# Cathoven-AI/Montreal-Forced-Aligner

Measured on AMD Instinct MI355X. Metric: aligned utterances/sec (whole node), 10 s utts, 5k-state triphone, higher is better.
Workload: dtype f32 scores from 2-way f16-split products (3*2^-22 per term worst case), f64 path costs

## Files before the change

montreal_forced_aligner_amd/csrc/feats.hip:

```cpp
#include <algorithm>
#include <cstdlib>

#include "ctx.hpp"

namespace {

constexpr int kTile = 64;
constexpr int kMaxDim = 16;
constexpr int kMaxOut = 64;
constexpr size_t kMaxLdsBytes = 64 << 10;

__global__ __launch_bounds__(256) void cmvn_utt_kernel(const float *__restrict__ feats, const int64_t *__restrict__ frame_off,
                                                       int dim, double *__restrict__ partial) {
  __shared__ double sx[16][kMaxDim], sxx[16][kMaxDim];
  const int utt = blockIdx.x, d = threadIdx.x & 15, s = threadIdx.x >> 4;
  const int64_t f0 = frame_off[utt];
  const int T = (int)(frame_off[utt + 1] - f0);
  double a = 0.0, b = 0.0;
  if (d < dim)
    for (int t = s; t < T; t += 16) {
      float x = feats[(f0 + t) * dim + d];
      a += (double)x;
      b += (double)(x * x);
    }
// ... 73 lines not shown
      int level = c / p.dim, d = c % p.dim;
      float acc = 0.0f;
      const float *xc = x + (r + halo) * p.dim + d;
      if (level == 0) acc = fmaf(1.0f, xc[0], acc);
      else if (level == 1) {
#pragma unroll
        for (int j = -2; j <= 2; j++) {
          int tf = t + j; tf = tf < 0 ? 0 : (tf >= T ? T - 1 : tf);
          float s = kDelta1[j + 2];
          if (s != 0.0f) acc = fmaf(s, xc[(tf - t) * p.dim], acc);
        }
      } else {
#pragma unroll
        for (int j = -4; j <= 4; j++) {
          int tf = t + j; tf = tf < 0 ? 0 : (tf >= T ? T - 1 : tf);
          float s = kDelta2[j + 4];
          if (s != 0.0f) acc = fmaf(s, xc[(tf - t) * p.dim], acc);
        }
      }
      p.out[(f0 + t) * od + c] = acc;
    }
    return;
  }
  const int nsp = 2 * p.ctx + 1, sdim = nsp * p.dim;
  const bool lda_offset = (p.lda_cols == sdim + 1);
  for (int i = threadIdx.x; i < kTile * p.lda_rows; i += blockDim.x) {
    int r = i / p.lda_rows, o = i % p.lda_rows, t = t0 + r;
    if (t >= T) continue;
    const float *m = mat + o * p.lda_cols;
    float acc = 0.0f;
    for (int j = 0; j < nsp; j++) {
      int tf = t + j - p.ctx; tf = tf < 0 ? 0 : (tf >= T ? T - 1 : tf);
      const float *xr = x + (tf - t0 + halo) * p.dim;
      for (int d = 0; d < p.dim; d++) acc = fmaf(m[j * p.dim + d], xr[d], acc);
    }
    if (lda_offset) acc += m[sdim];
    if (p.fmllr) y[r * p.lda_rows + o] = acc;
    else p.out[(f0 + t) * p.lda_rows + o] = acc;
  }
  if (!p.fmllr) return;
  __syncthreads();
  const float *fm = mat + p.lda_rows * p.lda_cols;
  for (int i = threadIdx.x; i < kTile * p.lda_rows; i += blockDim.x) {
    int r = i / p.lda_rows, o = i % p.lda_rows, t = t0 + r;
    if (t >= T) continue;
    const float *m = fm + o * (p.lda_rows + 1);
    float acc = 0.0f;
    for (int d = 0; d < p.lda_rows; d++) acc = fmaf(m[d], y[r * p.lda_rows + d], acc);
    acc += m[p.lda_rows];
    p.out[(f0 + t) * p.lda_rows + o] = acc;
  }
}

constexpr int kTileLda = 128;
template <int kDim, int kCtx, int kR>
__global__ __launch_bounds__(256) void feats_lda_kernel(FeatParams p) {
  extern __shared__ __attribute__((aligned(16))) float smem[];
  constexpr int kSdim = (2 * kCtx + 1) * kDim;
  constexpr int kXS = (kDim + 3) & ~3;
  static_assert(kR % 4 == 0, "LDA output rows are read 16 bytes at a time");
  const int utt = blockIdx.y;
  const int64_t f0 = p.frame_off[utt];
  const int T = (int)(p.frame_off[utt + 1] - f0);
  const int t0 = blockIdx.x * kTileLda;
  if (t0 >= T) return;
  constexpr int halo = kCtx, rows = kTileLda + 2 * halo;
  constexpr int R = kR;
  float *X = smem;
  constexpr int x_floats = rows * kXS > R * (R + 1) ? rows * kXS : R * (R + 1);
  float *Y = X + x_floats;
  const int spk = p.utt2spk ? p.utt2spk[utt] : 0;
  for (int i = threadIdx.x; i < rows * kDim; i += blockDim.x) {
    int r = i / kDim, d = i % kDim;
    int t = t0 - halo + r;
    t = t < 0 ? 0 : (t >= T ? T - 1 : t);
    float v = p.mfcc[(f0 + t) * kDim + d];
    if (p.cmvn) {
      const double *st = p.cmvn + (size_t)spk * 2 * (kDim + 1);
      v += (float)(-(st[d] / st[kDim]));
    }
    X[r * kXS + d] = v;
  }
  for (int i = threadIdx.x; i < R * p.lda_cols; i += blockDim.x) Y[i] = p.lda[i];
  __syncthreads();
  constexpr int G = 256 / R;
  const int o = threadIdx.x % R, g = threadIdx.x / R;
  const bool active = g < G;
  const bool lda_offset = (p.lda_cols == kSdim + 1);
  float m[kSdim];
#pragma unroll
  for (int k = 0; k < kSdim; k++) m[k] = Y[o * p.lda_cols + k];
  const float m_off = lda_offset ? Y[o * p.lda_cols + kSdim] : 0.0f;
  __syncthreads();
  if (active) {
    for (int r = g; r < kTileLda; r += 2 * G) {
      const int t = t0 + r;
      if (t >= T) break;
      const int r2 = r + G;
      const bool two = r2 < kTileLda && t0 + r2 < T;
      const float *xa = X + r * kXS;
      const float *xb = X + (two ? r2 : r) * kXS;
      float acc = 0.0f, acc2 = 0.0f;
#pragma unroll
      for (int j = 0; j < 2 * kCtx + 1; j++) {
        const float *xr = xa + j * kXS, *xr2 = xb + j * kXS;
#pragma unroll
        for (int d4 = 0; d4 + 4 <= kDim; d4 += 4) {
          const float4 x4 = *reinterpret_cast<const float4 *>(xr + d4);
          const float4 y4 = *reinterpret_cast<const float4 *>(xr2 + d4);
          acc = fmaf(m[j * kDim + d4], x4.x, acc);      acc2 = fmaf(m[j * kDim + d4], y4.x, acc2);
          acc = fmaf(m[j * kDim + d4 + 1], x4.y, acc);  acc2 = fmaf(m[j * kDim + d4 + 1], y4.y, acc2);
          acc = fmaf(m[j * kDim + d4 + 2], x4.z, acc);  acc2 = fmaf(m[j * kDim + d4 + 2], y4.z, acc2);
          acc = fmaf(m[j * kDim + d4 + 3], x4.w, acc);  acc2 = fmaf(m[j * kDim + d4 + 3], y4.w, acc2);
        }
#pragma unroll
        for (int d = kDim & ~3; d < kDim; d++) { acc = fmaf(m[j * kDim + d], xr[d], acc); acc2 = fmaf(m[j * kDim + d], xr2[d], acc2); }
      }
      if (lda_offset) { acc += m_off; acc2 += m_off; }
      if (p.fmllr) { Y[r * R + o] = acc; if (two) Y[r2 * R + o] = acc2; }
      else { p.out[(f0 + t) * R + o] = acc; if (two) p.out[(f0 + t0 + r2) * R + o] = acc2; }
    }
  }
  if (!p.fmllr) return;
  __syncthreads();
  const float *fm = p.fmllr + (size_t)spk * R * (R + 1);
  for (int i = threadIdx.x; i < R * (R + 1); i += blockDim.x) X[i] = fm[i];
  __syncthreads();
  if (!active) return;
  float f[kR];
#pragma unroll
  for (int k = 0; k < kR; k++) f[k] = X[o * (R + 1) + k];
  const float f_off = X[o * (R + 1) + R];
  for (int r = g; r < kTileLda; r += 2 * G) {
    const int t = t0 + r;
    if (t >= T) break;
    const int r2 = r + G;
    const bool two = r2 < kTileLda && t0 + r2 < T;
    const float *ys = Y + r * R, *ys2 = Y + (two ? r2 : r) * R;
    float acc = 0.0f, acc2 = 0.0f;
#pragma unroll
    for (int k = 0; k < kR; k += 4) {
      const float4 y4 = *reinterpret_cast<const float4 *>(ys + k);
      const float4 z4 = *reinterpret_cast<const float4 *>(ys2 + k);
      acc = fmaf(f[k], y4.x, acc);          acc2 = fmaf(f[k], z4.x, acc2);
      acc = fmaf(f[k + 1], y4.y, acc);      acc2 = fmaf(f[k + 1], z4.y, acc2);
      acc = fmaf(f[k + 2], y4.z, acc);      acc2 = fmaf(f[k + 2], z4.z, acc2);
      acc = fmaf(f[k + 3], y4.w, acc);      acc2 = fmaf(f[k + 3], z4.w, acc2);
    }
    acc += f_off; acc2 += f_off;
    p.out[(f0 + t) * R + o] = acc;
    if (two) p.out[(f0 + t0 + r2) * R + o] = acc2;
  }
}

int upload_delta_scales(mfa_ctx *c) {
  MFA_HIP_CHECK(c, hipSetDevice(c->device));
  float s0[1] = {1.0f}, s1[5] = {0}, s2[9] = {0};
  {
    float normalizer = 0.0f;
    for (int j = -2; j <= 2; j++) { normalizer += j * j; s1[j + 2] += (float)j * s0[0]; }
    float sc = (float)(1.0 / normalizer);
    for (float &v : s1) v *= sc;
  }
  {
    float normalizer = 0.0f;
    for (int j = -2; j <= 2; j++) {
      normalizer += j * j;
      for (int k = -2; k <= 2; k++) s2[j + k + 4] += (float)j * s1[k + 2];
    }
    float sc = (float)(1.0 / normalizer);
    for (float &v : s2) v *= sc;
  }
  MFA_HIP_CHECK(c, hipMemcpyToSymbol(HIP_SYMBOL(kDelta1), s1, sizeof(s1)));
  MFA_HIP_CHECK(c, hipMemcpyToSymbol(HIP_SYMBOL(kDelta2), s2, sizeof(s2)));
  return 0;
}

}

extern "C" {

MFA_API int mfa_cmvn_stats(mfa_ctx *c, const float *d_feats, const int64_t *d_frame_off, int32_t n_utt, int32_t dim,
                           const int32_t *d_spk_utt_off, const int32_t *d_spk_utt, int32_t n_spk, double *d_stats) {
  if (dim > kMaxDim) return c->fail("CMVN: feature dim %d > %d", dim, kMaxDim);
  if (n_utt <= 0 || n_spk <= 0) return 0;
  size_t need = (size_t)n_utt * 2 * (dim + 1) * sizeof(double);
  if (c->ws_bytes < need) {
    if (c->d_ws) { MFA_HIP_CHECK(c, hipStreamSynchronize(c->stream)); (void)hipFree(c->d_ws); c->d_ws = nullptr; c->ws_bytes = 0; }
    MFA_HIP_CHECK(c, hipMalloc(&c->d_ws, need));
    c->ws_bytes = need;
  }
  KernelTimer kt(c, MFA_K_CMVN);
  hipLaunchKernelGGL(cmvn_utt_kernel, dim3(n_utt), dim3(256), 0, c->stream, d_feats, d_frame_off, dim, (double *)c->d_ws);
  int total = n_spk * 2 * (dim + 1);
  hipLaunchKernelGGL(cmvn_spk_kernel, dim3((total + 255) / 256), dim3(256), 0, c->stream, (const double *)c->d_ws,
                     d_spk_utt_off, d_spk_utt, n_spk, dim, d_stats);
  MFA_HIP_CHECK(c, hipGetLastError());
  return 0;
}

MFA_API int mfa_feats_batch(mfa_ctx *c, const float *d_mfcc, const int64_t *d_frame_off, int32_t n_utt, int32_t max_frames,
                            int32_t dim, const int32_t *d_utt2spk, const double *d_cmvn, int32_t mode, int32_t splice_ctx,
                            const float *d_lda, int32_t lda_rows, int32_t lda_cols, const float *d_fmllr, float *d_out) {
  if (dim > kMaxDim) return c->fail("feats: base dim %d > %d", dim, kMaxDim);
  if (n_utt <= 0 || max_frames <= 0) return 0;
  if (n_utt > 65535) return c->fail("at most 65535 utterances per feature launch (got %d)", n_utt);
  if (mode != 0 && mode != 1) return c->fail("feats: bad mode %d", mode);
  if (d_cmvn && !d_utt2spk) return c->fail("feats: CMVN given without utt2spk");
  if (!c->delta_uploaded) { if (upload_delta_scales(c)) return -1; c->delta_uploaded = true; }
  FeatParams p;
  p.dim = dim; p.mode = mode; p.ctx = splice_ctx; p.lda_rows = lda_rows; p.lda_cols = lda_cols;
  p.mfcc = d_mfcc; p.frame_off = d_frame_off; p.utt2spk = d_utt2spk; p.cmvn = d_cmvn; p.lda = d_lda; p.fmllr = d_fmllr;
  p.out = d_out;
  constexpr int kDim = 13, kCtx = 3, kR = 40;
  const char *generic = getenv("MFA_FEATS_GENERIC");
  const bool register_rows = mode == 1 && dim == kDim && splice_ctx == kCtx && lda_rows == kR && !(generic && generic[0] == '1');
  size_t lds = 0;
  if (mode == 0) {
    lds = (size_t)(kTile + 8) * dim * 4;
  } else {
    int sdim = (2 * splice_ctx + 1) * dim;
    if (!d_lda || lda_rows <= 0 || lda_rows > kMaxOut || (lda_cols != sdim && lda_cols != sdim + 1))
      return c->fail("feats: LDA %dx%d does not match spliced dim %d", lda_rows, lda_cols, sdim);
    lds = ((size_t)(kTile + 2 * splice_ctx) * dim + (size_t)lda_rows * lda_cols + (size_t)lda_rows * (lda_rows + 1) +
           (size_t)kTile * lda_rows) * 4;
    if (lds > kMaxLdsBytes && !register_rows)
      return c->fail("feats: base dim %d, splice ±%d, LDA %dx%d needs %zu bytes of LDS (a launch may ask for %zu)", dim,
                     splice_ctx, lda_rows, lda_cols, lds, kMaxLdsBytes);
  }
  dim3 grid((max_frames + kTile - 1) / kTile, n_utt);
  KernelTimer kt(c, MFA_K_FEATS);
  if (register_rows) {
    const int rows = kTileLda + 2 * splice_ctx;
    size_t x_floats = std::max((size_t)rows * ((kDim + 3) & ~3), (size_t)lda_rows * (lda_rows + 1));
    size_t y_floats = std::max((size_t)kTileLda * lda_rows, (size_t)lda_rows * lda_cols);
    dim3 grid2((max_frames + kTileLda - 1) / kTileLda, n_utt);
    hipLaunchKernelGGL((feats_lda_kernel<kDim, kCtx, kR>), grid2, dim3(256), (x_floats + y_floats) * 4, c->stream, p);
  } else {
    hipLaunchKernelGGL(feats_kernel, grid, dim3(256), lds, c->stream, p);
  }
  MFA_HIP_CHECK(c, hipGetLastError());
  return 0;
}

}
```

montreal_forced_aligner_amd/csrc/viterbi.hip:

```cpp
#include <cmath>
#include <cstdint>
#include <cstdlib>
#include <cstring>

#include <algorithm>
#include <vector>

#include "ctx.hpp"

namespace {

typedef unsigned long long u64;
typedef unsigned int u32;

constexpr u32 kEmpty = 0xFFFFFFFFu;
constexpr u32 kClaim = 0xFFFFFFFEu;
constexpr u32 kOver = 0xFFFFFFFDu;
constexpr u64 kKeyInf = 0xFFFFFFFFFFFFFFFFull;
constexpr int kMinActive = 20;
constexpr float kBeamDelta = 0.5f;
constexpr float kHashRatio = 2.0f;
constexpr int kArcBits = 6;
constexpr int kMaxArcsPerState = 1 << kArcBits;

// ... 240 lines not shown
    }
  } else {
  {
    u32 pos = bpos;
    for (int c0 = T - 1; c0 >= 0; c0 -= 64) {
      const int tl = c0 - lane;
      const u32 tokv = tl >= 0 ? tokoff[tl] : 0u;
      const int cnt = min(64, c0 + 1);
      for (int k = 0; k < cnt; k++) {
        const u32 to = (u32)__builtin_amdgcn_readlane((int)tokv, k);
        const u64 rec = bp[(u64)to + pos];
        if (lane == 0) ali[c0 - k] = (int32_t)(rec >> 32);
        pos = (u32)(rec & 0xFFFFFFFFu);
      }
    }
  }
  __threadfence_block();
  WSYNC();
  for (int c0 = 0; c0 < T; c0 += 64) {
    const int tt = c0 + lane;
    int arc = tt < T ? ali[tt] : 0;
    int il = 0, ol = 0; float w = 0.0f, ac = 0.0f;
    if (tt < T) {
      il = a_il[arc]; ol = a_ol[arc]; w = a_w[arc];
      ac = -(p.scale * ll[(size_t)tt * P + a_col[arc]]);
    }
    const u64 mask = __ballot(ol != 0);
    if (ol != 0) words[nw_out + __popcll(mask & ((1ull << lane) - 1ull))] = ol;
    nw_out += (u32)__popcll(mask);
    float my_fl = 0.0f;
    const int lim = min(64, T - c0);
    for (int j = 0; j < lim; j++) {
      float wj = __shfl(w, j), acj = __shfl(ac, j);
      double nc = ((double)wj + cost) + (double)acj;
      float tot = (float)(nc - cost);
      float acost = tot - wj;
      w1 += wj; w2 += acost;
      cost = nc;
      if (lane == j) my_fl = acost * inv_scale;
    }
    if (tt < T) { ali[tt] = il; if (flike) flike[tt] = my_fl; }
  }
  }
  if (lane == 0) {
    w1 += final_w[fstate];
    p.like[utt] = -(w1 + w2) / p.scale;
    p.n_words[utt] = (int32_t)nw_out;
    p.status[utt] = p.pass == 0 ? ST_OK : ST_RETRIED;
  }
}

constexpr int kArcCache = 8;

template <bool kListsInLds, bool kEps = false>
__global__ __launch_bounds__(64) __attribute__((amdgpu_waves_per_eu(4, 4))) void viterbi_kernel(VitParams p) {
  extern __shared__ __attribute__((aligned(16))) unsigned char smem[];
  const int lane = threadIdx.x;
  int utt = blockIdx.x;
  if (p.utt_list) {
    if (p.n_list && (int)blockIdx.x >= *p.n_list) return;
    utt = p.utt_list[blockIdx.x];
  }
  const int64_t so = p.g.d_state_off[utt];
  const int S = (int)(p.g.d_state_off[utt + 1] - so);
  const int64_t ab_ = p.g.d_arc_base[utt];
  const int32_t *arc_off = p.g.d_arc_off + so + utt;
  const float *final_w = p.g.d_final + so;
  const float *a_w = p.g.d_arc_weight + ab_;
  const int32_t *a_col = p.g.d_arc_col + ab_;
  const uint4 *a_rec = p.w_arcnext + ab_;
  const int64_t f0 = p.frame_off[utt];
  const int T = (int)(p.frame_off[utt + 1] - f0);
  const float *ll = p.ll + p.ll_off[utt];
  const int P = p.ll_cols[utt];
  const int N = p.nmax, C = p.cmax;

  u64 *s_cost = (u64 *)smem;
  double *l_cost0 = kListsInLds ? (double *)(s_cost + N)
                                         : (double *)(p.w_cost + (size_t)utt * 2 * N);
  u32 *hmap = (u32 *)(s_cost + (kListsInLds ? 3 : 1) * (size_t)N);
  const bool hdirect = p.hbits == 0;
  const u32 HM = hdirect ? (u32)((S + 1) & ~1) : 1u << p.hbits, hmask = hdirect ? 0xFFFFFFFFu : HM - 1u;
  const int hshift = hdirect ? 0 : 32 - p.hbits;
  u32 *s_state = hmap + HM;
  u32 *s_F = s_state + N;
  u32 *s_W = s_F + N;
  u32 *s_aux = s_W + N;
  u32 *t_cbase = s_aux + N;
  u32 *s_an = t_cbase + N;
  u32 *s_bucket = s_an + N;
  u32 *l_state0 = kListsInLds ? s_bucket + N : (u32 *)(p.w_state + (size_t)utt * 2 * N);
  u32 *l_an0 = kListsInLds ? l_state0 + 2 * N : (u32 *)(p.w_state + (size_t)p.g.n_utt * 2 * N + (size_t)utt * 2 * N);
  u32 *cntord = s_bucket + N + (kListsInLds ? 4 * N : 0);
  float *ll_row = (float *)(cntord + C);
  u32 *ctr = (u32 *)(ll_row + p.llcap);
  u32 *bm = ctr + 4;
  u32 *e_pos = bm + kBmWords;
  u32 *e_inv = e_pos + N;
  u32 *e_arc = e_inv + N;
  u32 *e_tmp = e_arc + N;
  u32 *e_info = e_tmp + N;
  u32 *e_stk = e_info + N;
  if constexpr (kEps) {
    for (int i = lane; i < N; i += 64) e_tmp[i] = 0xFFFFFFFFu;
  }

  u32 *st_a = p.w_stash_a + (size_t)utt * C;
  u32 *st_b = p.w_stash_b + (size_t)utt * C;
  u64 *st_key = p.w_stash_key + (size_t)utt * C;
  u64 *bp = p.w_bp + (size_t)f0 * p.bpf;
  const u64 bp_cap = (u64)T * (u64)p.bpf;
  u32 *tokoff = p.w_tokoff + f0 + utt;

  for (u32 i = lane; i < HM; i += 64) hmap[i] = kEmpty;
// ... 56 lines not shown
              }
              who = nc_; nc_++; pushed = true;
            } else if (__longlong_as_double((long long)s_cost[found]) > ncst) {
              if (lane == 0) { s_cost[found] = (u64)__double_as_longlong(ncst); e_arc[found] = first + k; e_inv[found] = e; }
              who = found; pushed = true;
            }
            if (pushed) {
              if (sp >= 2u * (u32)N) { over = true; break; }
              if (lane == 0) e_stk[sp] = who;
              sp++;
            }
            WSYNC();
          }
        }
        if (over) status = ST_TOKEN_OVERFLOW;
        else {
          for (u32 c0 = 0; c0 < nc_; c0 += 64) {
            const u32 c_ = c0 + (u32)lane;
            if (c_ < nc_) {
              const u32 bc = s_state[c_] % H;
              u32 lead_c = c_;
              for (u32 x = 0; x < c_; x++) if (s_state[x] % H == bc) { lead_c = x; break; }
              u32 pos_ = 0;
              for (u32 x = 0; x < nc_; x++) {
                if (x == c_) continue;
                const u32 bx = s_state[x] % H;
                u32 lead_x = x;
                for (u32 y = 0; y < x; y++) if (s_state[y] % H == bx) { lead_x = y; break; }
                if (lead_x < lead_c || (lead_x == lead_c && x < c_)) pos_++;
              }
              e_pos[c_] = pos_;
            }
          }
          WSYNC();
          for (u32 c0 = 0; c0 < nc_; c0 += 64) {
            const u32 c_ = c0 + (u32)lane;
            if (c_ < nc_) {
              const u32 pos_ = e_pos[c_];
              l_state0[pos_] = s_state[c_];
              l_cost0[pos_] = __longlong_as_double((long long)s_cost[c_]);
              l_an0[pos_] = s_an[c_];
              bp[pos_] = ((u64)e_arc[c_] << 32) | (u64)(c_ == 0u ? 0u : e_pos[e_inv[c_]]);
            }
          }
          n = (int)nc_;
          bp_used = nc_;
          __threadfence_block();
          WSYNC();
        }
      }
    }
  } else {
    const VitState vs = p.w_vstate[utt];
    if (vs.done) return;
    n = vs.n; H = vs.H; bp_used = vs.bp_used; t = p.t_begin;
    if (n < 0 || n > N) { n = 0; status = ST_INTERNAL; }
    if (kListsInLds) {
      cur = 0;
      for (int i = lane; i < n; i += 64) { l_state0[i] = park_state[i]; l_an0[i] = park_an[i]; l_cost0[i] = park_cost[i]; }
    } else {
      cur = vs.cur & 1;
    }
  }
  const int t_stop = p.windowed ? min(T, p.t_end) : T;
  constexpr int kPre = 8;
  const bool row_cached = P <= p.llcap && P <= 64 * kPre;
  float pre[kPre];
#pragma unroll
  for (int r = 0; r < kPre; r++) pre[r] = (row_cached && t < T && lane + 64 * r < P) ? ll[(size_t)t * P + lane + 64 * r] : 0.0f;
  WSYNC();
  const bool spec = p.spec != 0 && p.windowed;
  if (spec) build_scored_bitmap(p, utt, lane, bm);
  bool viol = false;

#ifdef VIT_STAMPS
  unsigned long long stamp_acc[12] = {0}, stamp_last;
  asm volatile("s_memtime %0\n\ts_waitcnt lgkmcnt(0)" : "=s"(stamp_last)::"memory");
#endif
  for (; t < t_stop && status == ST_OK; t++) {
    const float *llt = ll + (size_t)t * P;
    auto stage_row = [&]() {
      if (row_cached) {
#pragma unroll
        for (int r = 0; r < kPre; r++) if (lane + 64 * r < P) ll_row[lane + 64 * r] = pre[r];
        WSYNC();
      }
    };
#ifdef VIT_STAMPS
    stamp_acc[10] += (unsigned long long)n;
    stamp_acc[11] += 1;
#endif
    STAMP(0);
    auto score = [&](int col) -> float {
      float v = ll_row[row_cached ? col : 0];
      if (!row_cached) v = *(const volatile float *)&llt[col];
      if (spec) viol |= !column_scored(bm, col);
      return v;
    };
    auto prefetch_next_row = [&]() {
      if (row_cached && t + 1 < t_stop) {
        const float *nx_row = llt + P;
#pragma unroll
        for (int r = 0; r < kPre; r++) if (lane + 64 * r < P) pre[r] = nx_row[lane + 64 * r];
      }
    };
    u32 *n_state = l_state0 + (cur ^ 1) * N;
    u32 *c_an = l_an0 + cur * N, *n_an = l_an0 + (cur ^ 1) * N;
// ... 443 lines not shown
            n_state[pos] = d;
            n_an[pos] = s_an[j];
            n_cost[pos] = dunkey(s_cost[j]);
            bp[bp_used + pos] = ((u64)arc << 32) | (u64)ppos;
          }
        }
      }
    }
    if (__any(broken)) { status = ST_INTERNAL; break; }
    WSYNC();
    for (u32 j0 = 0; j0 < nslots_f; j0 += 64) {
      u32 j = j0 + lane;
      if (j < nslots_f) { hmap[s_bucket[j]] = kEmpty; cntord[s_aux[j] & 0xFFFFFFu] = 0; }
    }
    if (lane == 0) { tokoff[t] = (u32)bp_used; ctr[0] = 0; ctr[1] = 0; }
    bp_used += nslots_f;
    n = (int)nslots_f;
    cur ^= 1;
    if (!kListsInLds) __threadfence_block();
    WSYNC();
    STAMP(8);
  }
#ifdef VIT_STAMPS
  if (lane == 0 && p.pass == 0 && p.stamps && p.utt_list == nullptr)
    for (int k = 0; k < 12; k++) p.stamps[(size_t)utt * 12 + k] += stamp_acc[k];
#endif
  __threadfence_block();
  u32 *c_state = l_state0 + cur * N;
  double *c_cost = l_cost0 + cur * N;
  if (p.windowed && status == ST_OK && t < T && n > 0) {
    const u32 *c_an = l_an0 + cur * N;
    u32 dmax = 0, dmin_inv = 0;
    for (int i = lane; i < n; i += 64) {
      const u32 s_ = c_state[i];
      if (kListsInLds) { park_state[i] = s_; park_an[i] = c_an[i]; park_cost[i] = c_cost[i]; }
      if (p.state_depth) {
        const int32_t *sd = p.state_depth + 2 * (so + (int64_t)s_);
        dmax = max(dmax, (u32)sd[0]);
        dmin_inv = max(dmin_inv, ~(u32)sd[1]);
      }
    }
    dmax = wave_max_u32(dmax);
    dmin_inv = wave_max_u32(dmin_inv);
    if (lane == 0) {
      VitState vs;
      vs.n = n; vs.cur = kListsInLds ? 0 : cur; vs.done = 0; vs.pad0 = 0; vs.H = H; vs.pad1 = 0; vs.bp_used = bp_used;
      p.w_vstate[utt] = vs;
      if (p.band) {
        const long long hi = (long long)dmax + (long long)p.next_window - 1;
        p.band[2 * utt] = p.state_depth ? (int32_t)~dmin_inv : 0;
        p.band[2 * utt + 1] = p.state_depth ? (int32_t)min(hi, (long long)INT32_MAX) : INT32_MAX;
      }
    }
    return;
  }
  if (p.windowed && lane == 0) {
    VitState vs;
    vs.n = 0; vs.cur = 0; vs.done = 1; vs.pad0 = 0; vs.H = H; vs.pad1 = 0; vs.bp_used = bp_used;
    p.w_vstate[utt] = vs;
  }
  if (p.pass == 0 && lane == 0) p.w_hash[utt] = H;

  finalize_utterance(p, utt, lane, status, t, T, n, c_state, c_cost, final_w, bp, tokoff, f0, ab_, a_w, a_col, ll, P, kEps, bp_used,
                     bp_cap);
}

constexpr int kSmallN = 64;
template <int kRounds, bool kEps = false>
__global__ __launch_bounds__(64) __attribute__((amdgpu_waves_per_eu(4, 8))) void viterbi_small_kernel(VitParams p) {
  extern __shared__ __attribute__((aligned(16))) unsigned char smem[];
  constexpr int N = kSmallN, C = 64 * kRounds;
  constexpr u32 HM = 256u, hmask = HM - 1u;
  constexpr int hshift = 24;
  const int lane = threadIdx.x;
  const int utt = blockIdx.x;
  const VitState vs0 = p.w_vstate[utt];
  const int K_ = p.t_end - p.t_begin;
  const int lag = (p.t_begin > 0 && vs0.pad0 != 0) ? 1 : 0;
  const int t_begin_u = p.t_begin - lag * K_;
  const bool resume = t_begin_u > 0;
  if (p.t_begin > 0 && vs0.done) return;
  const int64_t so = p.g.d_state_off[utt];
  const int S = (int)(p.g.d_state_off[utt + 1] - so);
  const int64_t ab_ = p.g.d_arc_base[utt];
  const int32_t *arc_off = p.g.d_arc_off + so + utt;
  const uint4 *a_rec = p.w_arcnext + ab_;
  const int64_t f0 = p.frame_off[utt];
  const int T = (int)(p.frame_off[utt + 1] - f0);
  const float *ll = p.ll + p.ll_off[utt];
  const int P = p.ll_cols[utt];
  u32 *park_state = p.w_state + (size_t)utt * 2 * N;
  u32 *park_an = p.w_state + (size_t)p.g.n_utt * 2 * N + (size_t)utt * 2 * N;
  double *park_cost = p.w_cost + (size_t)utt * 2 * N;
  auto hand_over = [&]() {
    if (lane != 0) return;
    VitState vs; vs.n = 0; vs.cur = 0; vs.done = 1; vs.pad0 = 0; vs.H = 1000u; vs.pad1 = 0; vs.bp_used = 0;
    p.w_vstate[utt] = vs;
    p.status[utt] = ST_GROW; p.n_words[utt] = 0; p.like[utt] = 0.0f;
  };

  int n = 1, t = 0;
  u32 H = 1000u;
  u64 bp_used = 0;
  const int start = p.g.d_start[utt];
  if (S <= 0 || start < 0 || start >= S || T <= 0) { hand_over(); return; }
  if (resume) {
    n = vs0.n; H = vs0.H; bp_used = vs0.bp_used; t = t_begin_u;
    if (n > N || n <= 0) { hand_over(); return; }
  }

  u64 *s_cost = (u64 *)smem;
  double *l_cost0 = (double *)(s_cost + N);
  u32 *hmap = (u32 *)(l_cost0 + 2 * N);
  u32 *s_state = hmap + HM;
  u32 *s_F = s_state + N;
  u32 *s_W = s_F + N;
  u32 *t_cbase = s_W + N;
// ... 611 lines not shown
}

MFA_API size_t mfa_align_workspace_bytes(mfa_ctx *c, int32_t n_utt, int64_t total_frames, const mfa_align_opts *o) {
  (void)c;
  int N = (o->max_tokens > 0 ? o->max_tokens : 1024) * 4, C = 8 * N;
  return ws_layout(n_utt, total_frames, N, C, o->bp_tokens_per_frame > 0 ? o->bp_tokens_per_frame : 512,
                   (int64_t)n_utt * 8 * N).total;
}

}

namespace {

int align_impl(mfa_ctx *c, const mfa_graph_batch *g, const float *d_loglikes, const int64_t *d_ll_off,
               const int32_t *d_ll_cols, const int64_t *d_frame_off, int64_t total_frames,
               int64_t total_arcs, int32_t max_states, int32_t max_arcs, const mfa_align_opts *o, int32_t *d_ali, int32_t *d_words, int32_t *d_n_words,
               float *d_like, float *d_frame_like, int32_t *d_status, const MfaLazyScoring *lazy) {
  MFA_HIP_CHECK(c, hipSetDevice(c->device));
  const int n_utt = g->n_utt;
  if (n_utt <= 0) return 0;
  if (o->beam <= 0.0f || (o->retry_beam != 0.0f && o->retry_beam <= o->beam))
    return c->fail("Beams do not make sense: beam %f, retry-beam %f", o->beam, o->retry_beam);
  if (max_states <= 0 || max_arcs <= 0) return c->fail("max_states and max_arcs must be positive");
  if (total_frames <= 0 || total_arcs <= 0) return c->fail("total_frames and total_arcs must be positive");
  if (max_arcs >= (1 << 25)) return c->fail("graphs with more than 2^25 arcs are not supported");
  const int bpf = o->bp_tokens_per_frame > 0 ? o->bp_tokens_per_frame : 512;
  const int passes = o->retry_beam != 0.0f ? 2 : 1;
  int N[2], C[2];
  for (int ps = 0; ps < 2; ps++) pick_caps(o, max_states, max_arcs, ps, &N[ps], &C[ps]);
  const int Nw = passes == 2 ? N[1] : N[0], Cw = passes == 2 ? C[1] : C[0];
  const bool eps = g->d_state_nemit != nullptr;
  if (eps && max_arcs >= (1 << 24)) return c->fail("graphs with epsilon arcs and more than 2^24 arcs are not supported");
  const int64_t eps_states = eps ? (int64_t)n_utt * max_states : 0;
  WsLayout w = ws_layout(n_utt, total_frames, Nw, Cw, bpf, total_arcs, eps_states);
  if (c->ws_bytes < w.total) {
    if (c->d_ws) { MFA_HIP_CHECK(c, hipStreamSynchronize(c->stream)); (void)hipFree(c->d_ws); c->d_ws = nullptr; c->ws_bytes = 0; }
    MFA_HIP_CHECK(c, hipMalloc(&c->d_ws, w.total));
    c->ws_bytes = w.total;
  }
  unsigned char *base = (unsigned char *)c->d_ws;
  hipLaunchKernelGGL(arcnext_kernel, dim3(n_utt), dim3(256), 0, c->stream, *g, (uint4 *)(base + w.arcnext),
                     eps ? (u32 *)(base + w.eps) : (u32 *)nullptr, max_states);
  if (lazy && mfa_gmm_presplit(c, lazy, d_frame_off, n_utt, total_frames) != 0) return -1;
  const int first_tier = lazy ? kSmallN : 128;
  int spec_slack = 0;
  if (lazy) {
    int look = lazy->window / 2;
    { const char *e = getenv("MFA_LAZY_LOOKAHEAD"); if (e && atoi(e) > 0) look = atoi(e); }
    spec_slack = std::max(0, lazy->window - 1 - look);
    if (lazy->plan.max_cols > 32 * kBmWords) spec_slack = 0;
  }
  int eps_pops_env = 0;
  { const char *e = getenv("MFA_VIT_EPS_POPS"); if (e && atoi(e) > 0) eps_pops_env = atoi(e); }
  struct Launch { int pass, N, C, code, grow; };
  std::vector<Launch> plan;
  if (N[0] > first_tier) {
    plan.push_back({0, first_tier, std::min(C[0], 4 * first_tier), 0, 1});
    plan.push_back({0, N[0], C[0], ST_GROW, 0});
  } else {
    plan.push_back({0, N[0], C[0], 0, 0});
  }
  if (passes == 2) plan.push_back({1, N[1], C[1], ST_PENDING, 0});
  for (Launch &L : plan) {
    const int ps = L.pass;
    const bool small_tier = lazy && L.grow;
    bool lists_in_lds = lds_bytes(max_states, L.N, L.C, true, eps) <= kLdsLimit / 2 ||
                        ((ps == 0 || L.code != 0) && lds_bytes(max_states, L.N, L.C, true, eps) <= kLdsLimit);
    while (lds_bytes(max_states, L.N, L.C, lists_in_lds, eps) > kLdsLimit && L.N > 64) {
      L.N = (L.N / 2 + 63) & ~63;
      if (L.C > 8 * L.N) L.C = 8 * L.N;
    }
    size_t lds = lds_bytes(max_states, L.N, L.C, lists_in_lds, eps);
    if (lds > kLdsLimit) return c->fail("Viterbi tables need %zu bytes of LDS (> 160 KiB): %d states, %d tokens", lds, max_states, L.N);
    VitParams p;
    memset(&p, 0, sizeof(p));
    p.g = *g; p.ll = d_loglikes; p.ll_off = d_ll_off; p.ll_cols = d_ll_cols; p.frame_off = d_frame_off;
    p.beam = ps == 0 ? o->beam : o->retry_beam; p.scale = o->acoustic_scale;
    p.nmax = L.N; p.cmax = L.C; p.bpf = bpf; p.pass = ps; p.grow = L.grow; p.hbits = hash_bits(max_states, L.N);
    WsLayout wp = ws_layout(n_utt, total_frames, L.N, L.C, bpf, total_arcs, eps_states);
    p.w_state = (u32 *)(base + wp.state); p.w_cost = (double *)(base + wp.cost);
    p.w_stash_a = (u32 *)(base + wp.sta); p.w_stash_b = (u32 *)(base + wp.stb); p.w_stash_key = (u64 *)(base + wp.stkey);
    p.w_bp = (u64 *)(base + wp.bp); p.w_tokoff = (u32 *)(base + wp.tokoff);
    p.w_hash = (u32 *)(base + w.hash);
    p.w_arcnext = (const uint4 *)(base + w.arcnext);
    p.w_epsinfo = eps ? (const u32 *)(base + w.eps) : nullptr; p.eps_stride = max_states;
    p.eps_pops = eps_pops_env ? eps_pops_env : 64 * L.N;
    p.llcap = kLlCap;
    p.stamps = (unsigned long long *)c->vit_stamps;
    p.utt_list = nullptr; p.n_list = nullptr;
    p.ali = d_ali; p.words = d_words; p.n_words = d_n_words; p.like = d_like; p.frame_like = d_frame_like; p.status = d_status;
    if (L.code != 0) {
      int32_t *d_list = (int32_t *)(base + w.list), *d_count = (int32_t *)(base + w.count);
      MFA_HIP_CHECK(c, hipMemsetAsync(d_count, 0, sizeof(int32_t), c->stream));
      hipLaunchKernelGGL(collect_pending_kernel, dim3((n_utt + 255) / 256), dim3(256), 0, c->stream, d_status, n_utt, L.code, d_list, d_count);
      p.utt_list = d_list; p.n_list = d_count;
    }
    p.windowed = 0; p.t_begin = 0; p.t_end = 0x7fffffff; p.next_window = 0;
    p.w_vstate = (VitState *)(base + w.vstate); p.state_depth = nullptr; p.band = nullptr;
    void (*k_lds)(VitParams) = eps ? viterbi_kernel<true, true> : viterbi_kernel<true, false>;
    void (*k_hbm)(VitParams) = eps ? viterbi_kernel<false, true> : viterbi_kernel<false, false>;
    MFA_HIP_CHECK(c, hipFuncSetAttribute((const void *)(lists_in_lds ? k_lds : k_hbm), hipFuncAttributeMaxDynamicSharedMemorySize, (int)lds));
    auto launch_decoder = [&]() {
      KernelTimer kt(c, MFA_K_VITERBI);
      if (lists_in_lds) hipLaunchKernelGGL(k_lds, dim3(n_utt), dim3(64), lds, c->stream, p);
      else hipLaunchKernelGGL(k_hbm, dim3(n_utt), dim3(64), lds, c->stream, p);
    };
    if (!lazy) {
      launch_decoder();
      MFA_DEBUG_POINT(c, "decoded pass=%d code=%d N=%d C=%d lds=%zu in_lds=%d", ps, L.code, L.N, L.C, lds, (int)lists_in_lds);
    } else {
      const int K = L.code == 0 ? lazy->window : std::max(lazy->window, 256);
      p.windowed = 1; p.next_window = K;
      p.state_depth = lazy->plan.d_state_depth; p.band = (int32_t *)(base + w.band);
      const bool spec = small_tier && spec_slack > 0;
      const int t_loop_end = lazy->max_frames + (small_tier ? K : 0);
      constexpr int kSmallRounds = 3;
      const size_t lds_small = (size_t)kSmallN * (8 + 16 + 6 * 4 + 8 + 8) + 256 * 4 + (size_t)64 * kSmallRounds * 4 + 16 + (size_t)kBmWords * 4 +
                               (eps ? (size_t)kSmallN * 7 * 4 : 0);
      for (int t0 = 0; t0 < t_loop_end; t0 += K) {
        MfaWindowScore ws;
        memset(&ws, 0, sizeof(ws));
        if (small_tier) { ws.lag = (const int32_t *)(base + w.vstate); ws.lag_stride = (int)(sizeof(VitState) / 4); ws.lag_word = 3; }
        ws.t_begin = t0; ws.window = K; ws.band = p.band; ws.utt_list = p.utt_list; ws.n_list = p.n_list;
        ws.cols_per_wave = L.code == 0 ? 0 : 32;
        ws.hi_slack = spec ? spec_slack : 0;
        ws.done = (const int32_t *)(base + w.vstate); ws.done_stride = (int)(sizeof(VitState) / 4); ws.done_word = 2;
        if (mfa_gmm_score_window(c, lazy, &ws, d_frame_off, n_utt, d_ll_off, (float *)d_loglikes) != 0) return -1;
        MFA_DEBUG_POINT(c, "scored window t0=%d K=%d pass=%d code=%d N=%d C=%d", t0, K, ps, L.code, L.N, L.C);
        p.t_begin = t0; p.t_end = t0 + K;
        p.spec = spec ? 1 : 0; p.spec_ranges = mfa_band_ranges(c); p.spec_class_counts = lazy->plan.d_class_counts;
        p.spec_groups = lazy->plan.groups;
        if (small_tier) {
          KernelTimer kt(c, MFA_K_VITERBI);
          if (eps) hipLaunchKernelGGL((viterbi_small_kernel<kSmallRounds, true>), dim3(n_utt), dim3(64), lds_small, c->stream, p);
          else hipLaunchKernelGGL((viterbi_small_kernel<kSmallRounds, false>), dim3(n_utt), dim3(64), lds_small, c->stream, p);
        } else {
          launch_decoder();
        }
        MFA_DEBUG_POINT(c, "decoded window t0=%d K=%d pass=%d code=%d N=%d C=%d lds=%zu in_lds=%d small=%d", t0, K, ps, L.code, L.N, L.C, lds,
                        (int)lists_in_lds, (int)small_tier);
      }
      if (small_tier) {
        KernelTimer kt(c, MFA_K_VITERBI);
        hipLaunchKernelGGL(viterbi_finish_kernel, dim3(n_utt), dim3(64), 0, c->stream, p);
      }
    }
    MFA_HIP_CHECK(c, hipGetLastError());
  }
  c->xsplit_ready = false;
  hipLaunchKernelGGL(finalize_pending_kernel, dim3((n_utt + 255) / 256), dim3(256), 0, c->stream, d_status, n_utt);
  MFA_HIP_CHECK(c, hipGetLastError());
  return 0;
}

}

extern "C" {

// ... 34 lines not shown
```

Baseline: 235,200.

## Compute spliced LDA and fMLLR feature transforms with MFMA f32 matrix instructions

Measured after the change: 236,000 (median of 4 runs). Within noise of the previous version (+0.3%).

```diff
diff --git a/montreal_forced_aligner_amd/csrc/feats.hip b/montreal_forced_aligner_amd/csrc/feats.hip
--- a/montreal_forced_aligner_amd/csrc/feats.hip
+++ b/montreal_forced_aligner_amd/csrc/feats.hip
@@ -149,104 +149,146 @@
   }
 }
 
-constexpr int kTileLda = 128;
+typedef float f32x4 __attribute__((ext_vector_type(4)));
+constexpr int kTileLda = 256;
+#define FEATS_WAVE_SYNC()                                        \
+  do {                                                           \
+    __builtin_amdgcn_fence(__ATOMIC_RELEASE, "wavefront");       \
+    __builtin_amdgcn_wave_barrier();                             \
+    __builtin_amdgcn_fence(__ATOMIC_ACQUIRE, "wavefront");       \
+  } while (0)
+template <int kDim, int kCtx, int kR> struct LdaShape {
+  static constexpr int kSdim = (2 * kCtx + 1) * kDim;
+  static constexpr int kRows = kTileLda + 2 * kCtx;
+  static constexpr int kXFloats = (kRows * kDim + 3) & ~3;
+  static constexpr int kYS = kR + 4;
+  static constexpr int kStage = kR * (kSdim + 1) + kR * (kR + 1);
+  static constexpr int kSFloats = kStage > 4 * 16 * kYS ? kStage : 4 * 16 * kYS;
+  static constexpr size_t kLdsBytes = (size_t)(kXFloats + kSFloats) * 4;
+};
 template <int kDim, int kCtx, int kR>
 __global__ __launch_bounds__(256) void feats_lda_kernel(FeatParams p) {
   extern __shared__ __attribute__((aligned(16))) float smem[];
-  constexpr int kSdim = (2 * kCtx + 1) * kDim;
-  constexpr int kXS = (kDim + 3) & ~3;
-  static_assert(kR % 4 == 0, "LDA output rows are read 16 bytes at a time");
+  using Sh = LdaShape<kDim, kCtx, kR>;
+  constexpr int kSdim = Sh::kSdim, kYS = Sh::kYS, R = kR;
+  constexpr int kKL = (kSdim + 3) / 4, kKF = kR / 4, kMT = (kR + 15) / 16;
+  static_assert(kR % 4 == 0, "a lane's four output rows are stored 16 bytes at a time");
+  __shared__ float s_off[kDim];
   const int utt = blockIdx.y;
   const int64_t f0 = p.frame_off[utt];
   const int T = (int)(p.frame_off[utt + 1] - f0);
   const int t0 = blockIdx.x * kTileLda;
   if (t0 >= T) return;
-  constexpr int halo = kCtx, rows = kTileLda + 2 * halo;
-  constexpr int R = kR;
   float *X = smem;
-  constexpr int x_floats = rows * kXS > R * (R + 1) ? rows * kXS : R * (R + 1);
-  float *Y = X + x_floats;
+  float *S = X + Sh::kXFloats;
   const int spk = p.utt2spk ? p.utt2spk[utt] : 0;
-  for (int i = threadIdx.x; i < rows * kDim; i += blockDim.x) {
+  if (p.cmvn && threadIdx.x < kDim) {
+    const double *st = p.cmvn + (size_t)spk * 2 * (kDim + 1);
+    s_off[threadIdx.x] = (float)(-(st[threadIdx.x] / st[kDim]));
+  }
+  float *SF = S + R * p.lda_cols;
+  for (int i = threadIdx.x; i < R * p.lda_cols; i += blockDim.x) S[i] = p.lda[i];
+  if (p.fmllr) {
+    const float *fm = p.fmllr + (size_t)spk * R * (R + 1);
+    for (int i = threadIdx.x; i < R * (R + 1); i += blockDim.x) SF[i] = fm[i];
+  }
+  __syncthreads();
+  for (int i = threadIdx.x; i < Sh::kRows * kDim; i += blockDim.x) {
     int r = i / kDim, d = i % kDim;
-    int t = t0 - halo + r;
+    int t = t0 - kCtx + r;
     t = t < 0 ? 0 : (t >= T ? T - 1 : t);
     float v = p.mfcc[(f0 + t) * kDim + d];
-    if (p.cmvn) {
-      const double *st = p.cmvn + (size_t)spk * 2 * (kDim + 1);
-      v += (float)(-(st[d] / st[kDim]));
-    }
-    X[r * kXS + d] = v;
-  }
-  for (int i = threadIdx.x; i < R * p.lda_cols; i += blockDim.x) Y[i] = p.lda[i];
-  __syncthreads();
-  constexpr int G = 256 / R;
-  const int o = threadIdx.x % R, g = threadIdx.x / R;
-  const bool active = g < G;
+    if (p.cmvn) v += s_off[d];
+    X[i] = v;
+  }
+  const int lane = threadIdx.x & 63, wave = threadIdx.x >> 6;
+  const int c = lane & 15, kq = lane >> 4;
   const bool lda_offset = (p.lda_cols == kSdim + 1);
-  float m[kSdim];
-#pragma unroll
-  for (int k = 0; k < kSdim; k++) m[k] = Y[o * p.lda_cols + k];
-  const float m_off = lda_offset ? Y[o * p.lda_cols + kSdim] : 0.0f;
-  __syncthreads();
-  if (active) {
-    for (int r = g; r < kTileLda; r += 2 * G) {
-      const int t = t0 + r;
-      if (t >= T) break;
-      const int r2 = r + G;
-      const bool two = r2 < kTileLda && t0 + r2 < T;
-      const float *xa = X + r * kXS;
-      const float *xb = X + (two ? r2 : r) * kXS;
-      float acc = 0.0f, acc2 = 0.0f;
-#pragma unroll
-      for (int j = 0; j < 2 * kCtx + 1; j++) {
-        const float *xr = xa + j * kXS, *xr2 = xb + j * kXS;
-#pragma unroll
-        for (int d4 = 0; d4 + 4 <= kDim; d4 += 4) {
-          const float4 x4 = *reinterpret_cast<const float4 *>(xr + d4);
-          const float4 y4 = *reinterpret_cast<const float4 *>(xr2 + d4);
-          acc = fmaf(m[j * kDim + d4], x4.x, acc);      acc2 = fmaf(m[j * kDim + d4], y4.x, acc2);
-          acc = fmaf(m[j * kDim + d4 + 1], x4.y, acc);  acc2 = fmaf(m[j * kDim + d4 + 1], y4.y, acc2);
-          acc = fmaf(m[j * kDim + d4 + 2], x4.z, acc);  acc2 = fmaf(m[j * kDim + d4 + 2], y4.z, acc2);
-          acc = fmaf(m[j * kDim + d4 + 3], x4.w, acc);  acc2 = fmaf(m[j * kDim + d4 + 3], y4.w, acc2);
-        }
-#pragma unroll
-        for (int d = kDim & ~3; d < kDim; d++) { acc = fmaf(m[j * kDim + d], xr[d], acc); acc2 = fmaf(m[j * kDim + d], xr2[d], acc2); }
+  float ml[kKL][kMT], mf[kKF][kMT];
+  f32x4 l_off[kMT], f_off[kMT];
+  const bool with_fmllr = p.fmllr != nullptr;
+#pragma unroll
+  for (int mt = 0; mt < kMT; mt++) {
+    const int o = 16 * mt + c;
+    const float *lrow = S + min(o, R - 1) * p.lda_cols, *frow = SF + min(o, R - 1) * (R + 1);
+#pragma unroll
+    for (int ks = 0; ks < kKL; ks++) {
+      const float v = lrow[min(4 * ks + kq, kSdim - 1)];
+      ml[ks][mt] = (o < R && 4 * ks + kq < kSdim) ? v : 0.0f;
+    }
+#pragma unroll
+    for (int ks = 0; ks < kKF; ks++) mf[ks][mt] = 0.0f;
+    if (with_fmllr) {
+#pragma unroll
+      for (int ks = 0; ks < kKF; ks++) {
+        const float v = frow[4 * ks + kq];
+        mf[ks][mt] = o < R ? v : 0.0f;
       }
-      if (lda_offset) { acc += m_off; acc2 += m_off; }
-      if (p.fmllr) { Y[r * R + o] = acc; if (two) Y[r2 * R + o] = acc2; }
-      else { p.out[(f0 + t) * R + o] = acc; if (two) p.out[(f0 + t0 + r2) * R + o] = acc2; }
-    }
-  }
-  if (!p.fmllr) return;
-  __syncthreads();
-  const float *fm = p.fmllr + (size_t)spk * R * (R + 1);
-  for (int i = threadIdx.x; i < R * (R + 1); i += blockDim.x) X[i] = fm[i];
-  __syncthreads();
-  if (!active) return;
-  float f[kR];
-#pragma unroll
-  for (int k = 0; k < kR; k++) f[k] = X[o * (R + 1) + k];
-  const float f_off = X[o * (R + 1) + R];
-  for (int r = g; r < kTileLda; r += 2 * G) {
-    const int t = t0 + r;
-    if (t >= T) break;
-    const int r2 = r + G;
-    const bool two = r2 < kTileLda && t0 + r2 < T;
-    const float *ys = Y + r * R, *ys2 = Y + (two ? r2 : r) * R;
-    float acc = 0.0f, acc2 = 0.0f;
-#pragma unroll
-    for (int k = 0; k < kR; k += 4) {
-      const float4 y4 = *reinterpret_cast<const float4 *>(ys + k);
-      const float4 z4 = *reinterpret_cast<const float4 *>(ys2 + k);
-      acc = fmaf(f[k], y4.x, acc);          acc2 = fmaf(f[k], z4.x, acc2);
-      acc = fmaf(f[k + 1], y4.y, acc);      acc2 = fmaf(f[k + 1], z4.y, acc2);
-      acc = fmaf(f[k + 2], y4.z, acc);      acc2 = fmaf(f[k + 2], z4.z, acc2);
-      acc = fmaf(f[k + 3], y4.w, acc);      acc2 = fmaf(f[k + 3], z4.w, acc2);
-    }
-    acc += f_off; acc2 += f_off;
-    p.out[(f0 + t) * R + o] = acc;
-    if (two) p.out[(f0 + t0 + r2) * R + o] = acc2;
+    }
+#pragma unroll
+    for (int e = 0; e < 4; e++) {
+      const int oe = 16 * mt + 4 * kq + e, oc = min(oe, R - 1);
+      const float lv = S[oc * p.lda_cols + p.lda_cols - 1];
+      l_off[mt][e] = (oe < R && lda_offset) ? lv : 0.0f;
+      f_off[mt][e] = 0.0f;
+      if (with_fmllr) { const float fv = SF[oc * (R + 1) + R]; f_off[mt][e] = oe < R ? fv : 0.0f; }
+    }
+  }
+  __syncthreads();
+  float *Y = S + wave * (16 * kYS);
+  const bool vec_out = (reinterpret_cast<uintptr_t>(p.out) & 15) == 0;
+  auto store = [&](int t, const f32x4 (&acc)[kMT]) {
+    float *dst = p.out + (f0 + t) * R + 4 * kq;
+#pragma unroll
+    for (int mt = 0; mt < kMT; mt++) {
+      if (16 * mt + 4 * kq >= R) continue;
+      if (vec_out) *reinterpret_cast<f32x4 *>(dst + 16 * mt) = acc[mt];
+      else { dst[16 * mt] = acc[mt][0]; dst[16 * mt + 1] = acc[mt][1]; dst[16 * mt + 2] = acc[mt][2]; dst[16 * mt + 3] = acc[mt][3]; }
+    }
+  };
+  for (int r0 = 16 * wave; r0 < kTileLda; r0 += 64) {
+    if (t0 + r0 >= T) break;
+    const int t = t0 + r0 + c;
+    const float *xs = X + (r0 + c) * kDim + kq;
+    f32x4 acc[kMT];
+#pragma unroll
+    for (int mt = 0; mt < kMT; mt++) acc[mt] = (f32x4){0.0f, 0.0f, 0.0f, 0.0f};
+    float b[kKL];
+#pragma unroll
+    for (int ks = 0; ks < kKL; ks++) b[ks] = (4 * ks + 3 < kSdim || 4 * ks + kq < kSdim) ? xs[4 * ks] : 0.0f;
+    __builtin_amdgcn_sched_barrier(0);
+#pragma unroll
+    for (int ks = 0; ks < kKL; ks++)
+#pragma unroll
+      for (int mt = 0; mt < kMT; mt++) acc[mt] = __builtin_amdgcn_mfma_f32_16x16x4f32(ml[ks][mt], b[ks], acc[mt], 0, 0, 0);
+    if (lda_offset) {
+#pragma unroll
+      for (int mt = 0; mt < kMT; mt++) acc[mt] += l_off[mt];
+    }
+    if (!with_fmllr) {
+      if (t < T) store(t, acc);
+      continue;
+    }
+#pragma unroll
+    for (int mt = 0; mt < kMT; mt++)
+      if (16 * mt + 4 * kq < R) *reinterpret_cast<f32x4 *>(Y + c * kYS + 16 * mt + 4 * kq) = acc[mt];
+    FEATS_WAVE_SYNC();
+    const float *ys = Y + c * kYS + kq;
+    f32x4 acc2[kMT];
+#pragma unroll
+    for (int mt = 0; mt < kMT; mt++) acc2[mt] = (f32x4){0.0f, 0.0f, 0.0f, 0.0f};
+    float b2[kKF];
+#pragma unroll
+    for (int ks = 0; ks < kKF; ks++) b2[ks] = ys[4 * ks];
+    __builtin_amdgcn_sched_barrier(0);
+#pragma unroll
+    for (int ks = 0; ks < kKF; ks++)
+#pragma unroll
+      for (int mt = 0; mt < kMT; mt++) acc2[mt] = __builtin_amdgcn_mfma_f32_16x16x4f32(mf[ks][mt], b2[ks], acc2[mt], 0, 0, 0);
+#pragma unroll
+    for (int mt = 0; mt < kMT; mt++) acc2[mt] += f_off[mt];
+    if (t < T) store(t, acc2);
+    FEATS_WAVE_SYNC();
   }
 }
 
@@ -328,11 +370,9 @@
   dim3 grid((max_frames + kTile - 1) / kTile, n_utt);
   KernelTimer kt(c, MFA_K_FEATS);
   if (register_rows) {
-    const int rows = kTileLda + 2 * splice_ctx;
-    size_t x_floats = std::max((size_t)rows * ((kDim + 3) & ~3), (size_t)lda_rows * (lda_rows + 1));
-    size_t y_floats = std::max((size_t)kTileLda * lda_rows, (size_t)lda_rows * lda_cols);
     dim3 grid2((max_frames + kTileLda - 1) / kTileLda, n_utt);
-    hipLaunchKernelGGL((feats_lda_kernel<kDim, kCtx, kR>), grid2, dim3(256), (x_floats + y_floats) * 4, c->stream, p);
+    constexpr size_t lds_lda = LdaShape<kDim, kCtx, kR>::kLdsBytes;
+    hipLaunchKernelGGL((feats_lda_kernel<kDim, kCtx, kR>), grid2, dim3(256), lds_lda, c->stream, p);
   } else {
     hipLaunchKernelGGL(feats_kernel, grid, dim3(256), lds, c->stream, p);
   }
```

## Use persistent grid-stride blocks for listed Viterbi retry/grow passes

Applied to the files above, without the earlier changes.

After: 235,500 before, 234,400 after. Within noise of the previous version (-0.5%).

```diff
diff --git a/montreal_forced_aligner_amd/csrc/viterbi.hip b/montreal_forced_aligner_amd/csrc/viterbi.hip
--- a/montreal_forced_aligner_amd/csrc/viterbi.hip
+++ b/montreal_forced_aligner_amd/csrc/viterbi.hip
@@ -316,14 +316,17 @@
 
 constexpr int kArcCache = 8;
 
-template <bool kListsInLds, bool kEps = false>
-__global__ __launch_bounds__(64) __attribute__((amdgpu_waves_per_eu(4, 4))) void viterbi_kernel(VitParams p) {
+template <bool kListsInLds, bool kEps = false, bool kList = false>
+__global__ __launch_bounds__(64) __attribute__((amdgpu_waves_per_eu(kList ? 1 : 4, kList ? 2 : 4))) void viterbi_kernel(VitParams p) {
   extern __shared__ __attribute__((aligned(16))) unsigned char smem[];
   const int lane = threadIdx.x;
-  int utt = blockIdx.x;
-  if (p.utt_list) {
-    if (p.n_list && (int)blockIdx.x >= *p.n_list) return;
-    utt = p.utt_list[blockIdx.x];
+#define NEXT_UTT() { if constexpr (kList) continue; else return; }
+  for (int li = blockIdx.x; ; li += gridDim.x) {
+  int utt = li;
+  if constexpr (kList) {
+    if (li >= *p.n_list) return;
+    utt = p.utt_list[li];
+    WSYNC();
   }
   const int64_t so = p.g.d_state_off[utt];
   const int S = (int)(p.g.d_state_off[utt + 1] - so);
@@ -486,7 +489,7 @@
     }
   } else {
     const VitState vs = p.w_vstate[utt];
-    if (vs.done) return;
+    if (vs.done) NEXT_UTT();
     n = vs.n; H = vs.H; bp_used = vs.bp_used; t = p.t_begin;
     if (n < 0 || n > N) { n = 0; status = ST_INTERNAL; }
     if (kListsInLds) {
@@ -1036,7 +1039,7 @@
         p.band[2 * utt + 1] = p.state_depth ? (int32_t)min(hi, (long long)INT32_MAX) : INT32_MAX;
       }
     }
-    return;
+    NEXT_UTT();
   }
   if (p.windowed && lane == 0) {
     VitState vs;
@@ -1047,6 +1050,9 @@
 
   finalize_utterance(p, utt, lane, status, t, T, n, c_state, c_cost, final_w, bp, tokoff, f0, ab_, a_w, a_col, ll, P, kEps, bp_used,
                      bp_cap);
+  if constexpr (!kList) return;
+  }
+#undef NEXT_UTT
 }
 
 constexpr int kSmallN = 64;
@@ -1764,6 +1770,8 @@
   }
   int eps_pops_env = 0;
   { const char *e = getenv("MFA_VIT_EPS_POPS"); if (e && atoi(e) > 0) eps_pops_env = atoi(e); }
+  int list_grid = 512;
+  { const char *e = getenv("MFA_VIT_LIST_GRID"); if (e && atoi(e) > 0) list_grid = atoi(e); }
   struct Launch { int pass, N, C, code, grow; };
   std::vector<Launch> plan;
   if (N[0] > first_tier) {
@@ -1809,13 +1817,17 @@
     }
     p.windowed = 0; p.t_begin = 0; p.t_end = 0x7fffffff; p.next_window = 0;
     p.w_vstate = (VitState *)(base + w.vstate); p.state_depth = nullptr; p.band = nullptr;
-    void (*k_lds)(VitParams) = eps ? viterbi_kernel<true, true> : viterbi_kernel<true, false>;
-    void (*k_hbm)(VitParams) = eps ? viterbi_kernel<false, true> : viterbi_kernel<false, false>;
+    const bool listed = L.code != 0;
+    void (*k_lds)(VitParams) = listed ? (eps ? viterbi_kernel<true, true, true> : viterbi_kernel<true, false, true>)
+                                      : (eps ? viterbi_kernel<true, true> : viterbi_kernel<true, false>);
+    void (*k_hbm)(VitParams) = listed ? (eps ? viterbi_kernel<false, true, true> : viterbi_kernel<false, false, true>)
+                                      : (eps ? viterbi_kernel<false, true> : viterbi_kernel<false, false>);
     MFA_HIP_CHECK(c, hipFuncSetAttribute((const void *)(lists_in_lds ? k_lds : k_hbm), hipFuncAttributeMaxDynamicSharedMemorySize, (int)lds));
+    const int grid = listed ? std::min(n_utt, list_grid) : n_utt;
     auto launch_decoder = [&]() {
       KernelTimer kt(c, MFA_K_VITERBI);
-      if (lists_in_lds) hipLaunchKernelGGL(k_lds, dim3(n_utt), dim3(64), lds, c->stream, p);
-      else hipLaunchKernelGGL(k_hbm, dim3(n_utt), dim3(64), lds, c->stream, p);
+      if (lists_in_lds) hipLaunchKernelGGL(k_lds, dim3(grid), dim3(64), lds, c->stream, p);
+      else hipLaunchKernelGGL(k_hbm, dim3(grid), dim3(64), lds, c->stream, p);
     };
     if (!lazy) {
       launch_decoder();
```
